# WangFeng18/3d-gaussian-splatting

Measured on NVIDIA H100. Metric: render+backward FPS @1080p (2.4M Gaussians), higher is better.
Workload: dtype f32

## Files before the change

3d-gaussian-splatting_b200/csrc/blend.cu:

```cuda
#include <cstdlib>
#include <type_traits>

#include "internal.h"

namespace {

constexpr int FWD_THREADS = 64;
constexpr int FWD_PX = 4;
constexpr int FWD_STAGES = 2;

template <int FWD_CH>
struct FwdSmem {
  float4 A[FWD_STAGES][FWD_CH];
  float4 C[FWD_STAGES][FWD_CH];
  float2 B[FWD_STAGES][FWD_CH + 2];
  uint64_t full[FWD_STAGES];
};

template <typename SM, int CH>
__device__ __forceinline__ void issue_chunk(SM& sm, int stage, const float4* __restrict__ pA,
                                            const float2* __restrict__ pB, const float4* __restrict__ pC,
                                            int base, int n, int shift) {
  uint32_t bytes_a = (uint32_t)n * 16u;
  uint32_t nb = (uint32_t)(n + shift + 1) & ~1u;
// ... 577 lines not shown
    const float ev = fmaf(-b.x * dy, dy, b.y);                                              \
    _Pragma("unroll") for (int p = 0; p < FWD_PX; ++p) {                                    \
      const float dx = px[p] - a.x;                                                         \
      const float eu = fmaf(a.z, dx, -m1);                                                  \
      const float alpha = gs_ex2(fmaf(-dx, eu, ev));                                        \
      const float w = (T[p] > GS_T_STOP) ? alpha * T[p] : 0.f;                              \
      cr[p] = fmaf(c.x, w, cr[p]);                                                          \
      cg[p] = fmaf(c.y, w, cg[p]);                                                          \
      cb[p] = fmaf(c.z, w, cb[p]);                                                          \
      T[p] -= w;                                                                            \
    }                                                                                       \
  }
    int j = 0;
    bool warp_dead = false;
    for (; j + 4 <= n; j += 4) {
#pragma unroll
      for (int u = 0; u < 4; ++u) GS_FWD_BODY(j + u)
      const bool dead = !(T[0] > GS_T_STOP) && !(T[1] > GS_T_STOP) && !(T[2] > GS_T_STOP) && !(T[3] > GS_T_STOP);
      if (__all_sync(0xffffffffu, dead)) {
        warp_dead = true;
        break;
      }
    }
    if (!warp_dead)
      for (; j < n; ++j) GS_FWD_BODY(j)
#undef GS_FWD_BODY
    const bool dead = !(T[0] > GS_T_STOP) && !(T[1] > GS_T_STOP) && !(T[2] > GS_T_STOP) && !(T[3] > GS_T_STOP);
    const int all_dead = gs_bar_red_and(1, WSF_CONS, dead);
    if (all_dead) {
      consumed = min(cnt, (k + 1) * WS_CH);
      if (tid == 0) {
        sm.consumed_chunks = k + 1;
        sm.stop = 1;
        gs_mbar_arrive(&sm.empty[stage]);
      }
      break;
    }
    if (tid == 0) {
      sm.consumed_chunks = k + 1;
      gs_mbar_arrive(&sm.empty[stage]);
    }
  }
  if (tid == 0 && nchunks > 0) gs_mbar_arrive(&sm.done);
  float4* o = reinterpret_cast<float4*>(image + ((size_t)iy * wp + ix0) * 3);
  o[0] = make_float4(cr[0], cg[0], cb[0], cr[1]);
  o[1] = make_float4(cg[1], cb[1], cr[2], cg[2]);
  o[2] = make_float4(cb[2], cr[3], cg[3], cb[3]);
  if (final_img) {
#pragma unroll
    for (int p = 0; p < FWD_PX; ++p)
      gs_store_final(final_img, ix0 + p, iy, crop.left, crop.top, crop.width, crop.height, cr[p], cg[p], cb[p]);
  }
  if (tile_neff && tid == 0) tile_neff[tile] = consumed;
}

template <int PX, int STAGES_, int RQ_>
struct Bwd2Cfg {
  static constexpr int NT = 256 / PX;
  static constexpr int TPR = GS_TILE / PX;
  static constexpr int RQ = RQ_;
  static constexpr int R = NT / RQ;
  static constexpr int SQ = NT / RQ;
  static constexpr int ROWS = SQ / TPR;
  static constexpr int QS = (SQ * 6 + 31) / 32 * 32 + 32 / RQ;
  static constexpr int IS = RQ * QS + 2 - (RQ * QS) % 32 + ((RQ * QS) % 32 > 2 ? 32 : 0);
  static constexpr int STAGES = STAGES_;
};

template <int PX, int STAGES, int RQ, bool GATHER, int CH>
struct Bwd2Smem : std::conditional<GATHER, GatherRing<CH, STAGES, 4>, WsRing<STAGES>>::type {
  float part[Bwd2Cfg<PX, STAGES, RQ>::R * Bwd2Cfg<PX, STAGES, RQ>::IS];
  float pyt[GS_TILE];
  int valid[2];
};

template <int PX, int STAGES, int RQ, bool GATHER, int CH>
struct Bwd2SmemAux : Bwd2Smem<PX, STAGES, RQ, GATHER, CH> {
  static constexpr int TQS = Bwd2Cfg<PX, STAGES, RQ>::SQ, TIS = Bwd2Cfg<PX, STAGES, RQ>::NT + 1;
  static_assert(Bwd2Cfg<PX, STAGES, RQ>::NT == 32 && TQS * RQ == 32 && TIS % 32 == 1,
                "d_t plane strides are conflict free for one consumer warp only");
  float part_t[Bwd2Cfg<PX, STAGES, RQ>::R * TIS];
};

template <int PX, bool AUX = false>
__device__ __forceinline__ void bwd_row(const float4 a, const float2 b, const float4 c, const float (&px)[PX],
                                        const float py, float (&T)[PX], float (&Rr)[PX], const float (&gr)[PX],
                                        const float (&gg)[PX], const float (&gb)[PX], float2* __restrict__ dst,
                                        const float t = 0.f, const float (*gD)[PX] = nullptr,
                                        const float (*gA)[PX] = nullptr, float* __restrict__ dst_t = nullptr) {
  float s0 = 0.f, sx = 0.f, sxx = 0.f, c0 = 0.f, c1 = 0.f, c2 = 0.f, dt = 0.f;
  const float dy = py - a.y;
  const float m1 = a.w * dy;
  const float ev = fmaf(-b.x * dy, dy, b.y);
#pragma unroll
  for (int p = 0; p < PX; ++p) {
    const float dx = px[p] - a.x;
    const float eu = fmaf(a.z, dx, -m1);
    float alpha = gs_ex2(fmaf(-dx, eu, ev));
    alpha = (T[p] > GS_T_STOP) ? alpha : 0.f;
    const float w = alpha * T[p];
    float gc = fmaf(gr[p], c.x, fmaf(gg[p], c.y, gb[p] * c.z));
    if constexpr (AUX) gc = fmaf((*gD)[p], t, gc + (*gA)[p]);
    Rr[p] = fmaf(-gc, w, Rr[p]);
    const float rc = gs_rcp(1.0000001f - alpha);
    const float dal = fmaf(T[p], gc, -Rr[p] * rc);
    const float e = dal * alpha;
    T[p] -= w;
    const float ex = e * dx;
    s0 += e;
    sx += ex;
    sxx = fmaf(ex, dx, sxx);
    c0 = fmaf(gr[p], w, c0);
    c1 = fmaf(gg[p], w, c1);
    c2 = fmaf(gb[p], w, c2);
    if constexpr (AUX) dt = fmaf((*gD)[p], w, dt);
  }
  dst[0] = make_float2(s0, sx);
  dst[1] = make_float2(sxx, c0);
  dst[2] = make_float2(c1, c2);
  if constexpr (AUX) *dst_t = dt;
}

template <int PX, bool WS, int UNR, int STAGES, int MINB, int RQ, bool GATHER, int CH, bool AUX = false>
__global__ void __launch_bounds__(256 / PX + (WS ? 32 : 0), MINB)
    blend_bwd2_kernel(const float4* __restrict__ pA, const float2* __restrict__ pB, const float4* __restrict__ pC,
                      const GsRec* __restrict__ grec, const uint32_t* __restrict__ ids,
                      const uint32_t* __restrict__ goff, const int* __restrict__ tile_accum, int wp, int hp, int ntx, float fx, float fy,
                      const float* __restrict__ image, const float* __restrict__ grad_image,
                      float* __restrict__ grad_inst, int grad_is_final, GsCrop crop, uint32_t* __restrict__ row_epoch,
                      uint32_t epoch, int* __restrict__ tile_neff_b, const float* __restrict__ aux,
                      const float* __restrict__ grad_aux) {
  using Cfg = Bwd2Cfg<PX, STAGES, RQ>;
  constexpr int NT = Cfg::NT, TPR = Cfg::TPR, R = Cfg::R, SQ = Cfg::SQ, QS = Cfg::QS, IS = Cfg::IS, ROWS = Cfg::ROWS;
  static_assert(IS % 2 == 0 && QS % 2 == 0 && IS % 32 == 2 && QS % 32 == 32 / RQ, "partial buffer strides");
  static_assert(!(WS && GATHER), "the gather path issues its copies from all consumer threads");
  static_assert(GATHER || CH == WS_CH, "the packed ring is sized for CH instances per stage");
  static_assert(!AUX || GATHER, "the aux terms read |p_c| from the gathered records");
  using Smem = typename std::conditional<AUX, Bwd2SmemAux<PX, STAGES, RQ, GATHER, CH>,
                                         Bwd2Smem<PX, STAGES, RQ, GATHER, CH>>::type;
  __shared__ __align__(16) Smem sm;
  const int tile = blockIdx.x;
  const int tid = threadIdx.x, warp = tid >> 5, lane = tid & 31;
  const int start = tile_accum[tile];
  const int cnt = tile_accum[tile + 1] - start;
  if (cnt == 0) return;
  const int nchunks = (cnt + CH - 1) / CH;
  const int tx = tile % ntx, ty = tile / ntx;
  const int shift = start & 1;
  if (tid < GS_TILE) sm.pyt[tid] = gs_pixel_coord(ty * GS_TILE + tid, hp, fy);
  if constexpr (GATHER) {
    if (tid == 0) {
      for (int s = 0; s < STAGES; ++s) gs_mbar_init(&sm.full[s], NT);
      gs_fence_barrier_init();
    }
    __syncthreads();
  } else {
    ws_init<Smem, STAGES>(sm, tid);
    if (WS) {
      if (tid >= NT) {
        if (tid == NT) ws_producer<Smem, STAGES>(sm, pA, pB, pC, start, cnt, nchunks);
        return;
      }
    } else if (tid == 0) {
      for (int k = 0; k < STAGES && k < nchunks; ++k)
        issue_chunk<Smem, CH>(sm, k, pA, pB, pC, start + k * CH, min(CH, cnt - k * CH), shift);
    }
  }
  GatherIds<NT, CH> gid;
  if constexpr (GATHER) {
    for (int k = 0; k < STAGES && k < nchunks; ++k) {
      gid.load(ids, start + k * CH, min(CH, cnt - k * CH), tid);
      gather_issue<Smem, NT, CH, 4>(sm, k, grec, goff, gid, min(CH, cnt - k * CH), tid);
    }
    if (STAGES < nchunks) gid.load(ids, start + STAGES * CH, min(CH, cnt - STAGES * CH), tid);
  }
  const int ix0 = tx * GS_TILE + (tid % TPR) * PX;
  const int iy = ty * GS_TILE + (tid / TPR);
  float px[PX];
#pragma unroll
  for (int p = 0; p < PX; ++p) px[p] = gs_pixel_coord(ix0 + p, wp, fx);
  const float py = sm.pyt[tid / TPR];

  float T[PX], Rr[PX], gr[PX], gg[PX], gb[PX];
  {
    const size_t off = ((size_t)iy * wp + ix0) * 3;
    const float4* im = reinterpret_cast<const float4*>(image + off);
    float gbuf[PX * 3], ibuf[PX * 3];
#pragma unroll
    for (int q = 0; q < PX * 3 / 4; ++q) {
      const float4 i4 = im[q];
      ibuf[4 * q] = i4.x; ibuf[4 * q + 1] = i4.y; ibuf[4 * q + 2] = i4.z; ibuf[4 * q + 3] = i4.w;
    }
    if (!grad_is_final) {
      const float4* gi = reinterpret_cast<const float4*>(grad_image + off);
#pragma unroll
      for (int q = 0; q < PX * 3 / 4; ++q) {
        const float4 g4 = gi[q];
        gbuf[4 * q] = g4.x; gbuf[4 * q + 1] = g4.y; gbuf[4 * q + 2] = g4.z; gbuf[4 * q + 3] = g4.w;
      }
    } else {
#pragma unroll
      for (int p = 0; p < PX; ++p)
        gs_load_final_grad(grad_image, ibuf + 3 * p, ix0 + p, iy, crop.left, crop.top, crop.width, crop.height,
                           gbuf[3 * p], gbuf[3 * p + 1], gbuf[3 * p + 2]);
    }
#pragma unroll
    for (int p = 0; p < PX; ++p) {
      gr[p] = gbuf[3 * p];
      gg[p] = gbuf[3 * p + 1];
      gb[p] = gbuf[3 * p + 2];
      Rr[p] = gr[p] * ibuf[3 * p] + gg[p] * ibuf[3 * p + 1] + gb[p] * ibuf[3 * p + 2];
      T[p] = 1.f;
    }
  }
  float gD[PX], gA[PX];
  if constexpr (AUX) {
    const size_t off = ((size_t)iy * wp + ix0) * 2;
    float abuf[PX * 2], gbuf[PX * 2];
#pragma unroll
    for (int q = 0; q < PX / 2; ++q) {
      const float4 v = reinterpret_cast<const float4*>(aux + off)[q];
      abuf[4 * q] = v.x; abuf[4 * q + 1] = v.y; abuf[4 * q + 2] = v.z; abuf[4 * q + 3] = v.w;
    }
    if (!grad_is_final) {
#pragma unroll
      for (int q = 0; q < PX / 2; ++q) {
        const float4 v = reinterpret_cast<const float4*>(grad_aux + off)[q];
        gbuf[4 * q] = v.x; gbuf[4 * q + 1] = v.y; gbuf[4 * q + 2] = v.z; gbuf[4 * q + 3] = v.w;
      }
    } else {
#pragma unroll
      for (int p = 0; p < PX; ++p) {
        const int x = ix0 + p - crop.left, y = iy - crop.top;
        float2 v = make_float2(0.f, 0.f);
        if (x >= 0 && x < crop.width && y >= 0 && y < crop.height)
          v = *reinterpret_cast<const float2*>(grad_aux + ((size_t)y * crop.width + x) * 2);
        gbuf[2 * p] = v.x;
        gbuf[2 * p + 1] = v.y;
      }
    }
#pragma unroll
    for (int p = 0; p < PX; ++p) {
      gD[p] = gbuf[2 * p];
      gA[p] = gbuf[2 * p + 1];
      Rr[p] = fmaf(gD[p], abuf[2 * p], fmaf(gA[p], abuf[2 * p + 1], Rr[p]));
    }
  }
  float2* const my_part = reinterpret_cast<float2*>(sm.part + (tid / SQ) * QS + (tid % SQ) * 6);
  float* my_part_t = nullptr;
  if constexpr (AUX) my_part_t = sm.part_t + (tid / SQ) * Smem::TQS + (tid % SQ);
  const int ri = tid / RQ, rq = tid % RQ;
  const float2* const red_src = reinterpret_cast<const float2*>(sm.part + ri * IS + rq * QS);

  int consumed = cnt;
  bool finished = false;
  int k = 0;
  for (; k < nchunks && !finished; ++k) {
    const int stage = k % STAGES;
    gs_mbar_wait(&sm.full[stage], (uint32_t)((k / STAGES) & 1));
    const int n = min(CH, cnt - k * CH);
    StageView<GATHER> sv;
    if constexpr (GATHER) {
      sv.R = sm.rec[stage];
      sv.recw = 4;
    } else {
      sv.A = sm.A[stage];
      sv.C = sm.C[stage];
      sv.B = sm.B[stage] + shift;
    }

    for (int sub = 0; sub < n; sub += R) {
      const int nr = min(R, n - sub);
      int j = 0;
      bool wdead = false;
      for (; j + UNR <= nr; j += UNR) {
        if (UNR >= 4 || (j & 3) == 0) {
          bool dead = true;
#pragma unroll
          for (int p = 0; p < PX; ++p) dead = dead && !(T[p] > GS_T_STOP);
          if (__all_sync(0xffffffffu, dead)) {
            wdead = true;
            break;
          }
        }
#pragma unroll
        for (int u = 0; u < UNR; ++u) {
          if constexpr (AUX)
            bwd_row<PX, true>(sv.a(sub + j + u), sv.b(sub + j + u), sv.c(sub + j + u), px, py, T, Rr, gr, gg, gb,
                              my_part + (j + u) * (IS / 2), sv.depth(sub + j + u), &gD, &gA,
                              my_part_t + (j + u) * Smem::TIS);
          else
            bwd_row<PX>(sv.a(sub + j + u), sv.b(sub + j + u), sv.c(sub + j + u), px, py, T, Rr, gr, gg, gb,
                        my_part + (j + u) * (IS / 2));
        }
      }
      if (UNR > 1 && !wdead)
        for (; j < nr; ++j) {
          if constexpr (AUX)
            bwd_row<PX, true>(sv.a(sub + j), sv.b(sub + j), sv.c(sub + j), px, py, T, Rr, gr, gg, gb,
                              my_part + j * (IS / 2), sv.depth(sub + j), &gD, &gA, my_part_t + j * Smem::TIS);
          else
            bwd_row<PX>(sv.a(sub + j), sv.b(sub + j), sv.c(sub + j), px, py, T, Rr, gr, gg, gb, my_part + j * (IS / 2));
        }
      bool dead = true;
#pragma unroll
      for (int p = 0; p < PX; ++p) dead = dead && !(T[p] > GS_T_STOP);
      int all_dead;
      int v0, v1;
      if (NT == 64) {
        if (lane == 0) sm.valid[warp] = j;
        all_dead = gs_bar_red_and(1, NT, dead);
        v0 = sm.valid[0];
        v1 = sm.valid[1];
      } else {
        __syncwarp();
        all_dead = __all_sync(0xffffffffu, dead);
        v0 = v1 = j;
      }
      {
        float S0 = 0.f, Sx = 0.f, Sxx = 0.f, Sy = 0.f, Sxy = 0.f, Syy = 0.f, C0 = 0.f, C1 = 0.f, C2 = 0.f;
        const bool act = ri < nr;
        float4 a = make_float4(0.f, 0.f, 0.f, 0.f);
        float2 b = make_float2(0.f, 0.f);
        if (act) {
          a = sv.a(sub + ri);
          b = sv.b(sub + ri);
        }
        const int vq = (NT == 64 && rq * SQ >= 32) ? v1 : v0;
        if (act && ri < vq) {
#pragma unroll
          for (int r = 0; r < ROWS; ++r) {
            float2 u0 = red_src[(r * TPR) * 3], u1 = red_src[(r * TPR) * 3 + 1], u2 = red_src[(r * TPR) * 3 + 2];
#pragma unroll
            for (int t = 1; t < TPR; ++t) {
              const float2 w0 = red_src[(r * TPR + t) * 3], w1 = red_src[(r * TPR + t) * 3 + 1],
                           w2 = red_src[(r * TPR + t) * 3 + 2];
              u0.x += w0.x; u0.y += w0.y; u1.x += w1.x; u1.y += w1.y; u2.x += w2.x; u2.y += w2.y;
            }
            const float dyr = sm.pyt[ROWS * rq + r] - a.y;
            S0 += u0.x;
            Sx += u0.y;
            Sxx += u1.x;
            C0 += u1.y;
            C1 += u2.x;
            C2 += u2.y;
            Sy = fmaf(dyr, u0.x, Sy);
            Sxy = fmaf(dyr, u0.y, Sxy);
            Syy = fmaf(dyr * dyr, u0.x, Syy);
          }
        }
        float Dt = 0.f;
        if constexpr (AUX) {
          if (act && ri < vq) {
            const float* src = sm.part_t + ri * Smem::TIS + rq * Smem::TQS;
#pragma unroll
            for (int s = 0; s < SQ; ++s) Dt += src[s];
          }
        }
#define GS_RED4(V)                                   \
  V += __shfl_xor_sync(0xffffffffu, V, 1);           \
  V += __shfl_xor_sync(0xffffffffu, V, 2);           \
  if (RQ == 8) V += __shfl_xor_sync(0xffffffffu, V, 4);
        GS_RED4(S0) GS_RED4(Sx) GS_RED4(Sxx) GS_RED4(Sy) GS_RED4(Sxy) GS_RED4(Syy) GS_RED4(C0) GS_RED4(C1) GS_RED4(C2)
        if constexpr (AUX) { GS_RED4(Dt) }
#undef GS_RED4
        if (act) {
          const uint32_t slot = sv.slot(sub + ri, tx, ty);
          float4* out = reinterpret_cast<float4*>(grad_inst + (size_t)slot * GS_GREC);
          if (rq == 0)
            out[0] = make_float4(GS_LN2 * (2.f * a.z * Sx - a.w * Sy), GS_LN2 * (2.f * b.x * Sy - a.w * Sx),
                                 -GS_LN2 * Sxx, GS_LN2 * Sxy);
          else if (rq == 1)
            out[1] = make_float4(-GS_LN2 * Syy, GS_LN2 * S0, C0, C1);
          else if (rq == 2)
            out[2] = make_float4(C2, Dt, 0.f, 0.f);
          else if (rq == 3 && row_epoch)
            row_epoch[slot] = epoch;
        }
      }
      if (NT == 64) gs_bar_sync(1, NT);
      else __syncwarp();
      if (all_dead) {
        consumed = min(cnt, k * CH + sub + nr);
        finished = true;
        break;
      }
    }
    if constexpr (GATHER) {
      if (!finished && k + STAGES < nchunks) {
        const int kn = k + STAGES;
        gather_issue<Smem, NT, CH, 4>(sm, stage, grec, goff, gid, min(CH, cnt - kn * CH), tid);
        if (kn + 1 < nchunks) gid.load(ids, start + (kn + 1) * CH, min(CH, cnt - (kn + 1) * CH), tid);
      }
    } else if (tid == 0) {
      if (WS) {
        sm.consumed_chunks = k + 1;
        if (finished) sm.stop = 1;
        gs_mbar_arrive(&sm.empty[stage]);
      } else if (!finished && k + STAGES < nchunks) {
        const int kn = k + STAGES;
        issue_chunk<Smem, CH>(sm, stage, pA, pB, pC, start + kn * CH, min(CH, cnt - kn * CH), shift);
      }
    }
  }
  if (tid == 0) {
    if constexpr (!GATHER && WS) {
      gs_mbar_arrive(&sm.done);
    } else if (finished) {
      for (int kk = k; kk < nchunks && kk < k + STAGES - 1; ++kk)
        gs_mbar_wait(&sm.full[kk % STAGES], (uint32_t)((kk / STAGES) & 1));
    }
    if (tile_neff_b) tile_neff_b[tile] = consumed;
  }
  if (row_epoch || GATHER) return;
  for (int t = consumed + tid; t < cnt; t += NT) {
    const uint32_t slot = __float_as_uint(pC[start + t].w);
    float4* out = reinterpret_cast<float4*>(grad_inst + (size_t)slot * GS_GREC);
    const float4 z = make_float4(0.f, 0.f, 0.f, 0.f);
    out[0] = z;
    out[1] = z;
    out[2] = z;
  }
}

__global__ void __launch_bounds__(256) legacy_pack_kernel(const float* __restrict__ pos, const float* __restrict__ rgb,
                                                           const float* __restrict__ opa,
                                                           const float* __restrict__ cov, int m,
                                                           float4* __restrict__ pA, float2* __restrict__ pB,
                                                           float4* __restrict__ pC) {
  int i = blockIdx.x * 256 + threadIdx.x;
  if (i >= m) return;
  float4 cv = reinterpret_cast<const float4*>(cov)[i];
  GsConic k = gs_make_conic(cv.x, cv.y, cv.z, cv.w);
  pA[i] = make_float4(pos[3 * i], pos[3 * i + 1], k.ca, k.cb);
  pB[i] = make_float2(k.cc, log2f(opa[i]));
  pC[i] = make_float4(rgb[3 * i], rgb[3 * i + 1], rgb[3 * i + 2], __uint_as_float((uint32_t)i));
}

__global__ void __launch_bounds__(256) legacy_unpack_grads_kernel(const float* __restrict__ grad_inst,
                                                                   const float* __restrict__ opa,
                                                                   const float* __restrict__ cov, int m,
                                                                   float* __restrict__ g_pos,
                                                                   float* __restrict__ g_rgb,
                                                                   float* __restrict__ g_opa,
                                                                   float* __restrict__ g_cov) {
  int i = blockIdx.x * 256 + threadIdx.x;
  if (i >= m) return;
  const float4* row = reinterpret_cast<const float4*>(grad_inst + (size_t)i * GS_GREC);
  float4 v0 = row[0], v1 = row[1], v2 = row[2];
  float4 cv = reinterpret_cast<const float4*>(cov)[i];
  float det = cv.x * cv.w - cv.y * cv.z;
  double pn = 2.0 * (double)det + 1e-14;
  float sc = (float)((double)GS_LOG2E / pn);
  float kk = 2.f * sc * sc / GS_LOG2E;
  float gsc = v0.z * cv.w + v0.w * (cv.y + cv.z) + v1.x * cv.x;
  g_pos[3 * i] = v0.x;
  g_pos[3 * i + 1] = v0.y;
  reinterpret_cast<float4*>(g_cov)[i] = make_float4(v1.x * sc - gsc * kk * cv.w, v0.w * sc + gsc * kk * cv.z,
                                                    v0.w * sc + gsc * kk * cv.y, v0.z * sc - gsc * kk * cv.x);
  g_opa[i] = opa[i] > 0.f ? v1.y / (opa[i] * GS_LN2) : 0.f;
  g_rgb[3 * i] = v1.z;
  g_rgb[3 * i + 1] = v1.w;
  g_rgb[3 * i + 2] = v2.x;
}

__global__ void __launch_bounds__(256) legacy_pack_sh_kernel(const float* __restrict__ pos,
                                                              const float* __restrict__ rgb,
                                                              const float* __restrict__ opa,
                                                              const float* __restrict__ cov, int m, int d, int sw,
// ... 28 lines not shown
  float kk = 2.f * sc * sc / GS_LOG2E;
  float d_ca = row[2], d_cb = row[3], d_cc = row[4];
  float gsc = d_ca * cv.w + d_cb * (cv.y + cv.z) + d_cc * cv.x;
  g_pos[3 * i] = row[0];
  g_pos[3 * i + 1] = row[1];
  reinterpret_cast<float4*>(g_cov)[i] = make_float4(d_cc * sc - gsc * kk * cv.w, d_cb * sc + gsc * kk * cv.z,
                                                    d_cb * sc + gsc * kk * cv.y, d_ca * sc - gsc * kk * cv.x);
  g_opa[i] = opa[i] > 0.f ? row[5] / (opa[i] * GS_LN2) : 0.f;
  for (int q = 0; q < d; ++q) g_rgb[(size_t)i * d + q] = row[6 + q];
}

struct LegacyWs {
  float4* pA;
  float2* pB;
  float4* pC;
  float* grad_inst;
};

inline size_t align_up(size_t x, size_t a) { return (x + a - 1) / a * a; }

inline size_t legacy_ws_layout(int m, int d, LegacyWs* ws, char* base) {
  size_t off = 0;
  size_t mm = (size_t)(m > 0 ? m : 0);
  size_t crow = d == 3 ? 16 : (size_t)gs_sh_stream_width(d) * 4;
  size_t grow = d == 3 ? (size_t)GS_GREC * 4 : (size_t)gs_sh_grad_width(d) * 4;
  if (ws) ws->pA = reinterpret_cast<float4*>(base + off);
  off += align_up(mm * 16, 256);
  if (ws) ws->pC = reinterpret_cast<float4*>(base + off);
  off += align_up(mm * crow + 16, 256);
  if (ws) ws->pB = reinterpret_cast<float2*>(base + off);
  off += align_up((mm + 2) * 8, 256);
  if (ws) ws->grad_inst = reinterpret_cast<float*>(base + off);
  off += align_up(mm * grow, 256);
  return off;
}

}

cudaError_t gs_launch_blend_fwd(const float4* pA, const float2* pB, const float4* pC, const GsRec* grec,
                                const uint32_t* ids, const int* tile_accum, const GsFrameGeom& g, float* image,
                                int* tile_neff, float* final_img, const GsCrop& crop, cudaStream_t st,
                                const GsAuxOut* aux) {
  const GsTuning& tn = gs_tuning();
  const bool gather = grec != nullptr;
  if (aux) {
    blend_fwd_kernel<128, 4, true, true><<<g.n_tiles, 64, 0, st>>>(pA, pB, pC, grec, ids, tile_accum, g.wp, g.hp, g.ntx,
                                                                  g.fx, g.fy, image, tile_neff, final_img, crop, *aux);
    return cudaGetLastError();
  }
  if (!gather && tn.fwd_kernel != 0) {
    blend_fwd_ws_kernel<<<g.n_tiles, WSF_CONS + 32, 0, st>>>(pA, pB, pC, tile_accum, g.wp, g.hp, g.ntx, g.fx, g.fy, image,
                                                             tile_neff, final_img, crop);
    return cudaGetLastError();
  }
  const int ch = tn.fwd_ch;
#define GS_FWD_LAUNCH(CH, PX, GA)                                                                                   \
  blend_fwd_kernel<CH, PX, GA><<<g.n_tiles, 256 / PX, 0, st>>>(pA, pB, pC, grec, ids, tile_accum, g.wp, g.hp, g.ntx, \
                                                               g.fx, g.fy, image, tile_neff, final_img, crop, GsAuxOut{})
#define GS_FWD_CH(PX, GA)                     \
  if (ch == 64) GS_FWD_LAUNCH(64, PX, GA);    \
  else if (ch == 256) GS_FWD_LAUNCH(256, PX, GA); \
  else GS_FWD_LAUNCH(128, PX, GA)
  if (gather) {
    if (tn.fwd_px == 8) { GS_FWD_CH(8, true); } else { GS_FWD_CH(4, true); }
  } else {
    if (tn.fwd_px == 8) { GS_FWD_CH(8, false); } else { GS_FWD_CH(4, false); }
  }
#undef GS_FWD_CH
#undef GS_FWD_LAUNCH
  return cudaGetLastError();
}

cudaError_t gs_launch_blend_bwd(const float4* pA, const float2* pB, const float4* pC, const GsRec* grec,
                                const uint32_t* ids, const uint32_t* goff, const int* tile_accum, const GsFrameGeom& g,
                                const float* image,
                                const float* grad_image, float* grad_inst, int grad_is_final, const GsCrop& crop,
                                uint32_t* row_epoch, uint32_t epoch, int* tile_neff_b, cudaStream_t st,
                                const float* aux, const float* grad_aux) {
  const GsTuning& tn = gs_tuning();
  const bool gather = grec != nullptr;
  if (gather && !row_epoch) return cudaErrorInvalidValue;
  if (grad_aux) {
    if (!gather || !aux) return cudaErrorInvalidValue;
    blend_bwd2_kernel<8, false, 4, 3, 10, 4, true, 32, true><<<g.n_tiles, 32, 0, st>>>(
        pA, pB, pC, grec, ids, goff, tile_accum, g.wp, g.hp, g.ntx, g.fx, g.fy, image, grad_image, grad_inst,
        grad_is_final, crop, row_epoch, epoch, tile_neff_b, aux, grad_aux);
    return cudaGetLastError();
  }
  if (tn.bwd_kernel != 0 || gather) {
#define GS_BWD2C(PX, WS, UNR, ST, MINB, RQ, GA, CH)                                                                 \
  blend_bwd2_kernel<PX, WS, UNR, ST, MINB, RQ, GA, CH><<<g.n_tiles, 256 / PX + (WS ? 32 : 0), 0, st>>>(              \
      pA, pB, pC, grec, ids, goff, tile_accum, g.wp, g.hp, g.ntx, g.fx, g.fy, image, grad_image, grad_inst,          \
      grad_is_final,                                                                                                 \
      crop, row_epoch, epoch, tile_neff_b, nullptr, nullptr)
#define GS_BWD2(PX, WS, UNR, ST, MINB, RQ, GA) GS_BWD2C(PX, WS, UNR, ST, MINB, RQ, GA, 64)
    const int key = ((((tn.bwd_px * 10 + tn.bwd_ws) * 10 + tn.bwd_unroll) * 10 + tn.bwd_stages) * 10 + tn.bwd_rq) * 100 +
                    tn.bwd_minb;
    if (gather && tn.bwd_ch == 32) {
      switch (key) {
        case 8022416: GS_BWD2C(8, false, 2, 2, 16, 4, true, 32); break;
        case 8023416: GS_BWD2C(8, false, 2, 3, 16, 4, true, 32); break;
        case 8042410: GS_BWD2C(8, false, 4, 2, 10, 4, true, 32); break;
        case 8043410: GS_BWD2C(8, false, 4, 3, 10, 4, true, 32); break;
        default: return gs_tuning().strict ? cudaErrorInvalidValue : (GS_BWD2C(8, false, 4, 3, 10, 4, true, 32), cudaGetLastError());
      }
      return cudaGetLastError();
    }
    if (gather) {
      switch (key) {
        case 8012410: GS_BWD2(8, false, 1, 2, 10, 4, true); break;
        case 8022416: GS_BWD2(8, false, 2, 2, 16, 4, true); break;
        case 8022410: GS_BWD2(8, false, 2, 2, 10, 4, true); break;
        case 8042410: GS_BWD2(8, false, 4, 2, 10, 4, true); break;
        case 8023416: GS_BWD2(8, false, 2, 3, 16, 4, true); break;
        case 8012416: GS_BWD2(8, false, 1, 2, 16, 4, true); break;
        case 8012420: GS_BWD2(8, false, 1, 2, 20, 4, true); break;
        case 8012820: GS_BWD2(8, false, 1, 2, 20, 8, true); break;
        case 8013416: GS_BWD2(8, false, 1, 3, 16, 4, true); break;
        case 4012401: GS_BWD2(4, false, 1, 2, 1, 4, true); break;
        case 4042401: GS_BWD2(4, false, 4, 2, 1, 4, true); break;
        default: return gs_tuning().strict ? cudaErrorInvalidValue : (GS_BWD2(8, false, 2, 2, 16, 4, true), cudaGetLastError());
      }
      return cudaGetLastError();
    }
    switch (key) {
      case 4113401: GS_BWD2(4, true, 1, 3, 1, 4, false); break;
      case 4143408: GS_BWD2(4, true, 4, 3, 8, 4, false); break;
      case 4012401: GS_BWD2(4, false, 1, 2, 1, 4, false); break;
      case 4042401: GS_BWD2(4, false, 4, 2, 1, 4, false); break;
      case 4042810: GS_BWD2(4, false, 4, 2, 10, 8, false); break;
      case 8012410: GS_BWD2(8, false, 1, 2, 10, 4, false); break;
      case 8012416: GS_BWD2(8, false, 1, 2, 16, 4, false); break;
      case 8012420: GS_BWD2(8, false, 1, 2, 20, 4, false); break;
      case 8013416: GS_BWD2(8, false, 1, 3, 16, 4, false); break;
      case 8022416: GS_BWD2(8, false, 2, 2, 16, 4, false); break;
      case 8022410: GS_BWD2(8, false, 2, 2, 10, 4, false); break;
      case 8042410: GS_BWD2(8, false, 4, 2, 10, 4, false); break;
      case 8012816: GS_BWD2(8, false, 1, 2, 16, 8, false); break;
      case 8012820: GS_BWD2(8, false, 1, 2, 20, 8, false); break;
      case 8112410: GS_BWD2(8, true, 1, 2, 10, 4, false); break;
      case 8012424: GS_BWD2(8, false, 1, 2, 24, 4, false); break;
      case 8012824: GS_BWD2(8, false, 1, 2, 24, 8, false); break;
      default: return gs_tuning().strict ? cudaErrorInvalidValue : (GS_BWD2(8, false, 2, 2, 16, 4, false), cudaGetLastError());
    }
#undef GS_BWD2
#undef GS_BWD2C
    return cudaGetLastError();
  }
  const int warps = tn.bwd_px == 8 ? 1 : 2;
  const int ch = 64;
#define GS_BWD_LAUNCH(W, CH)                                                                                         \
  blend_bwd_kernel<W, CH><<<g.n_tiles, 32 * W, 0, st>>>(pA, pB, pC, tile_accum, g.wp, g.hp, g.ntx, g.fx, g.fy, image, \
                                                        grad_image, grad_inst, grad_is_final, crop, row_epoch, epoch, \
                                                        tile_neff_b)
  if (warps == 1) GS_BWD_LAUNCH(1, 64);
  else if (ch == 32) GS_BWD_LAUNCH(2, 32);
  else if (ch == 128) GS_BWD_LAUNCH(2, 128);
  else GS_BWD_LAUNCH(2, 64);
#undef GS_BWD_LAUNCH
  return cudaGetLastError();
}

int gs_blend_aux_supported(int d, bool forward, bool backward) {
  const GsTuning& tn = gs_tuning();
  if (!tn.gather)
    return gs_set_error_msg(GS_ERR_UNSUPPORTED, "depth / alpha / background: the packed path (gs_tune(\"gather\", 0)) has no aux kernel");
  if (d != 3) {
    if (backward && (gs_sh_tc_mode(d) & 6) == 6)
      return gs_set_error_msg(GS_ERR_UNSUPPORTED,
                              "depth / alpha gradients: the two-pixel tensor-core SH backward (sh_tc bit 2) has no aux kernel");
    return 0;
  }
  if (forward && (tn.fwd_kernel != 0 || tn.fwd_ch != 128 || tn.fwd_px != 4))
    return gs_set_error_msg(GS_ERR_UNSUPPORTED,
                            "depth / alpha / background: only the shipped forward blend knobs (fwd_kernel 0, fwd_ch 128, fwd_px 4) have an aux kernel");
  if (backward && (tn.bwd_kernel == 0 || tn.bwd_px != 8 || tn.bwd_ws != 0 || tn.bwd_unroll != 4 || tn.bwd_stages != 3 ||
                   tn.bwd_rq != 4 || tn.bwd_minb != 10 || tn.bwd_ch != 32))
    return gs_set_error_msg(GS_ERR_UNSUPPORTED,
                            "depth / alpha gradients: only the shipped backward blend knobs have an aux kernel");
  return 0;
}

extern "C" size_t gs_draw_workspace_bytes(int m, int d) {
  if (d != 3 && gs_sh_basis_count(d) == 0) return 0;
  return legacy_ws_layout(m, d, nullptr, nullptr);
}

static int check_draw_args(const char* fn, int m, int d, int wp, int hp, int weight_normalize, int sigmoid,
// ... 102 lines not shown
```

3d-gaussian-splatting_b200/csrc/internal.h:

```cpp
#pragma once
#include <cuda_runtime.h>
#include <stdint.h>

#include "../../include/gs_b200.h"
#include "project.cuh"

#define GS_GREC 12

struct GsFrameGeom {
  int width, height, wp, hp, ntx, nty, n_tiles;
  float fx, fy;
};

struct GsCrop {
  int left, top, width, height;
};

struct GsAuxOut {
  float bg[3];
  float* aux;
  float* aux_final;
};

#ifdef __CUDACC__
__device__ __forceinline__ void gs_store_aux(const GsAuxOut& ax, int ix, int iy, int wp, const GsCrop& crop,
                                             float depth, float alpha) {
  if (ax.aux) *reinterpret_cast<float2*>(ax.aux + ((size_t)iy * wp + ix) * 2) = make_float2(depth, alpha);
  const int x = ix - crop.left, y = iy - crop.top;
  if (ax.aux_final && x >= 0 && x < crop.width && y >= 0 && y < crop.height)
    *reinterpret_cast<float2*>(ax.aux_final + ((size_t)y * crop.width + x) * 2) = make_float2(depth, alpha);
}
template <int PX>
__device__ __forceinline__ void gs_load_aux_grad(const float* __restrict__ aux, const float* __restrict__ grad_aux,
                                                 int grad_is_final, int ix0, int iy, int wp, const GsCrop& crop,
                                                 float (&gD)[PX], float (&gA)[PX], float (&R)[PX]) {
#pragma unroll
  for (int p = 0; p < PX; ++p) {
    const size_t off = ((size_t)iy * wp + ix0 + p) * 2;
    const float2 da = *reinterpret_cast<const float2*>(aux + off);
    float2 g = make_float2(0.f, 0.f);
    if (!grad_is_final) {
      g = *reinterpret_cast<const float2*>(grad_aux + off);
    } else {
      const int x = ix0 + p - crop.left, y = iy - crop.top;
      if (x >= 0 && x < crop.width && y >= 0 && y < crop.height)
        g = *reinterpret_cast<const float2*>(grad_aux + ((size_t)y * crop.width + x) * 2);
    }
    gD[p] = g.x;
    gA[p] = g.y;
    R[p] = fmaf(g.x, da.x, fmaf(g.y, da.y, R[p]));
  }
}
#endif

struct GsRayPtrs {
  const float *rays_o, *lefttop, *dx, *dy;
};

struct GsTuning {
  int fwd_kernel;
  int fwd_ch;
  int bwd_kernel;
  int bwd_px;
  int bwd_ws;
  int bwd_unroll;
  int bwd_stages;
  int bwd_minb;
  int bwd_rq;
  int fwd_px;
  int bwd_ch;
  int strict;
  int gather;
  int sh_tc;
};
GsTuning& gs_tuning();

void gs_count_launch(int n = 1);

int gs_sh_basis_count(int d);
int gs_sh_stream_width(int d);
int gs_sh_grad_width(int d);
int gs_sh_tc_mode(int d);
cudaError_t gs_launch_blend_sh_fwd(const float4* pA, const float2* pB, const float* pS, const GsRec* grec,
                                   const float* rgb, const uint32_t* ids, const uint32_t* goff , int d,
                                   const int* tile_accum,
                                   const GsFrameGeom& g, const GsRayPtrs& r, float* image, int* tile_neff,
                                   float* final_img, const GsCrop& crop, cudaStream_t st,
                                   const GsAuxOut* aux = nullptr );
cudaError_t gs_launch_blend_sh_bwd(const float4* pA, const float2* pB, const float* pS, const GsRec* grec,
                                   const float* rgb, const uint32_t* ids, const uint32_t* goff , int d,
                                   const int* tile_accum,
                                   const GsFrameGeom& g, const GsRayPtrs& r, const float* image,
                                   const float* grad_image, float* grad_inst, int grad_is_final, const GsCrop& crop,
                                   uint32_t* row_epoch, uint32_t epoch, int* tile_neff_b, cudaStream_t st,
                                   const float* aux = nullptr, const float* grad_aux = nullptr );

cudaError_t gs_launch_blend_sh_fwd_tc(const GsRec* grec, const float* rgb, const uint32_t* ids, int d,
                                      const int* tile_accum, const GsFrameGeom& g, const GsRayPtrs& r, float* image,
                                      int* tile_neff, float* final_img, const GsCrop& crop, cudaStream_t st,
                                      const GsAuxOut* aux = nullptr);
cudaError_t gs_launch_blend_sh_bwd_tc(const GsRec* grec, const float* rgb, const uint32_t* ids, const uint32_t* goff, int d,
                                      const int* tile_accum, const GsFrameGeom& g, const GsRayPtrs& r, const float* image,
                                      const float* grad_image, float* grad_inst, int grad_is_final, const GsCrop& crop,
                                      uint32_t* row_epoch, uint32_t epoch, int* tile_neff_b, cudaStream_t st,
                                      const float* aux = nullptr, const float* grad_aux = nullptr);

cudaError_t gs_launch_fused_project(const float* pos, const float* rgb, const float* opa, const float* quat,
                                    const float* scale, int n, int d, int scale_act, const GsCam& cam,
                                    const GsTileGrid& grid, float near_plane, float half_w, float half_h,
                                    GsRec* rec, uint32_t* count, uint32_t* dkey, int64_t* mask,
                                    unsigned int* n_visible, cudaStream_t st,
                                    bool sh_gaussian = false );

struct GsGradPush {
  float* bucket;
  float* staging[GS_MAX_PEERS];
  uint32_t per;
  int rank, world;
};

cudaError_t gs_launch_fused_project_bwd(const float* pos, const float* rgb, const float* opa, const float* quat,
                                        const float* scale, int n, int d, int scale_act, const GsCam& cam,
                                        float near_plane, float half_w, float half_h, const uint32_t* offsets_g,
                                        const uint32_t* count, const float* grad_inst, const uint32_t* row_epoch, uint32_t epoch,
                                        float* g_pos, float* g_rgb, float* g_opa,
                                        float* g_quat, float* g_scale, const GsGradPush& push, cudaStream_t st,
                                        bool depth_grad = false ,
                                        bool sh_gaussian = false );
size_t gs_cam_grad_workspace_bytes(int n);
cudaError_t gs_launch_fused_project_bwd_cam(const float* pos, const float* rgb, const float* opa, const float* quat,
                                            const float* scale, int n, int d, int scale_act, const GsCam& cam,
                                            float near_plane, float half_w, float half_h, const uint32_t* offsets_g,
                                            const uint32_t* count, const float* grad_inst, const uint32_t* row_epoch,
                                            uint32_t epoch, float* g_pos, float* g_rgb, float* g_opa, float* g_quat,
                                            float* g_scale, float* cam_part, float* grad_cam, cudaStream_t st,
                                            bool depth_grad, bool sh_gaussian);

cudaError_t gs_launch_emit_keys(const GsRec* rec, const uint32_t* perm, const uint32_t* offsets_sorted, int n, int ntx,
                                void* keys, int key_bytes, uint32_t* vals, cudaStream_t st);
cudaError_t gs_launch_tile_ranges(const void* keys, int key_bytes, long long m, int n_tiles, int* tile_accum,
                                  cudaStream_t st);

cudaError_t gs_launch_pack_sorted(const void* keys, int key_bytes, const uint32_t* vals, long long m, int n_tiles,
                                  int ntx, const GsRec* rec, const uint32_t* offsets_g, float4* pA, float2* pB, float4* pC,
                                  int* tile_accum, cudaStream_t st);

cudaError_t gs_launch_pack_sorted_sh(const void* keys, int key_bytes, const uint32_t* vals, long long m, int n_tiles,
                                     int ntx, const GsRec* rec, const uint32_t* offsets_g, const float* rgb, int d, int sw,
                                     float4* pA, float2* pB, float* pS, int* tile_accum, cudaStream_t st);
cudaError_t gs_launch_iota(uint32_t* out, int n, cudaStream_t st);

cudaError_t gs_launch_blend_fwd(const float4* pA, const float2* pB, const float4* pC, const GsRec* grec,
                                const uint32_t* ids, const int* tile_accum, const GsFrameGeom& g, float* image,
                                int* tile_neff, float* final_img, const GsCrop& crop, cudaStream_t st,
                                const GsAuxOut* aux = nullptr );

// ... 10 lines not shown
```

3d-gaussian-splatting_b200/csrc/render.cu:

```cuda
#include <cub/device/device_radix_sort.cuh>
#include <cub/device/device_scan.cuh>
#include <cub/iterator/counting_input_iterator.cuh>
#include <cub/iterator/transform_input_iterator.cuh>

#include <cmath>
#include <cstdio>
#include <cstdlib>
#include <cstring>
#include <new>

#include "internal.h"

struct GsCountInSortedOrder {
  const uint32_t* count;
  const uint32_t* perm;
  uint32_t n;
  __host__ __device__ __forceinline__ uint32_t operator()(uint32_t i) const { return i < n ? count[perm[i]] : 0u; }
};

static thread_local char g_err[512] = {0};

int gs_set_error(cudaError_t e, const char* what) {
  snprintf(g_err, sizeof(g_err), "CUDA error %d (%s) at %s", (int)e, cudaGetErrorString(e), what);
  return (int)e;
}
int gs_set_error_msg(int code, const char* what) {
  snprintf(g_err, sizeof(g_err), "%s", what);
  return code;
}
extern "C" const char* gs_last_error(void) { return g_err; }
extern "C" int gs_abi_version(void) { return 2; }

static int tune_env(const char* name, int dflt) {
  const char* e = getenv(name);
  return e ? atoi(e) : dflt;
}
GsTuning& gs_tuning() {
  static GsTuning t = {tune_env("GS_TUNE_FWD_KERNEL", 0),  tune_env("GS_TUNE_FWD_CH", 128),   tune_env("GS_TUNE_BWD_KERNEL", 1),
                       tune_env("GS_TUNE_BWD_PX", 8),      tune_env("GS_TUNE_BWD_WS", 0),     tune_env("GS_TUNE_BWD_UNROLL", 4),
                       tune_env("GS_TUNE_BWD_STAGES", 3),  tune_env("GS_TUNE_BWD_MINB", 10),  tune_env("GS_TUNE_BWD_RQ", 4),
                       tune_env("GS_TUNE_FWD_PX", 4),      tune_env("GS_TUNE_BWD_CH", 32),    tune_env("GS_TUNE_STRICT", 0),
                       tune_env("GS_TUNE_GATHER", 1),      tune_env("GS_TUNE_SH_TC", -1)};
  return t;
}
extern "C" int gs_tune(const char* name, int value) {
  if (!name) return gs_set_error_msg(GS_ERR_INVALID_ARG, "gs_tune: null name");
  GsTuning& t = gs_tuning();
  struct { const char* k; int* v; } tab[] = {{"fwd_kernel", &t.fwd_kernel}, {"fwd_ch", &t.fwd_ch},
                                             {"bwd_kernel", &t.bwd_kernel}, {"bwd_px", &t.bwd_px},
                                             {"bwd_ws", &t.bwd_ws},         {"bwd_unroll", &t.bwd_unroll},
                                             {"bwd_stages", &t.bwd_stages}, {"bwd_minb", &t.bwd_minb},
                                             {"bwd_rq", &t.bwd_rq},         {"fwd_px", &t.fwd_px},
                                             {"gather", &t.gather},         {"bwd_ch", &t.bwd_ch},
                                             {"strict", &t.strict},         {"sh_tc", &t.sh_tc}};
  for (auto& e : tab)
    if (!strcmp(e.k, name)) {
      *e.v = value;
      return 0;
    }
  return gs_set_error_msg(GS_ERR_INVALID_ARG, "gs_tune: unknown knob");
}

#include <atomic>
static std::atomic<unsigned long long> g_launches{0};
void gs_count_launch(int n) { g_launches.fetch_add((unsigned long long)n, std::memory_order_relaxed); }
extern "C" unsigned long long gs_kernel_launches(void) { return g_launches.load(std::memory_order_relaxed); }

struct GsAllocator {
  gs_alloc_fn alloc = nullptr;
  gs_free_fn free = nullptr;
  void* user = nullptr;
};
static thread_local const GsAllocator* g_cur_alloc = nullptr;

struct DevBuf {
  void* p = nullptr;
  size_t cap = 0;
  const GsAllocator* owner = nullptr;
  void drop(cudaStream_t st, bool sync) {
    if (!p) return;
    if (owner && owner->free) {
      owner->free(p, owner->user);
    } else {
      if (sync) cudaStreamSynchronize(st);
      cudaFree(p);
    }
    p = nullptr;
    cap = 0;
  }
  cudaError_t reserve(size_t bytes, cudaStream_t st) {
    if (bytes <= cap) return cudaSuccess;
    drop(st, true);
    size_t want = bytes + bytes / 8 + 256;
    const GsAllocator* a = g_cur_alloc;
    if (a && a->alloc) {
      p = a->alloc(want, a->user, (gs_stream_t)st);
      if (!p) return cudaErrorMemoryAllocation;
      owner = a;
    } else {
      cudaError_t e = cudaMalloc(&p, want);
      if (e != cudaSuccess) return e;
      owner = nullptr;
    }
    cap = want;
    return cudaSuccess;
  }
  void release() { drop(nullptr, false); }
  template <typename T>
  T* as() const { return static_cast<T*>(p); }
};

struct gs_ctx {
  int device = 0;
  GsAllocator allocator{};
  DevBuf rec, count, offsets, dkey_in, dkey_out, perm, iota, offsets_g;
  size_t iota_n = 0;
  DevBuf keys_in, keys_out, vals_in, vals_out, pA, pB, pC, grad_inst, row_epoch;
  uint32_t epoch = 0;
  DevBuf tile_accum, tile_neff, tile_neff_b, cub_tmp, counters, img_dev, gimg_dev, rays;
  DevBuf cam_part;
  float* host_rays = nullptr;
  unsigned long long* host_m = nullptr;
  cudaEvent_t ev_m = nullptr;
  bool have_forward = false, have_backward = false, gather = false;
  bool have_aux = false;
  bool sh_gaussian = false;
  int n = 0, d = 3, scale_act = 0;
  long long m = 0;
  GsCam cam{};
  GsTileGrid grid{};
  GsFrameGeom geom{};
  float near_plane = 0.f, half_w = 0.f, half_h = 0.f;
  int64_t* mask_ptr = nullptr;
  bool timing = false;
  cudaEvent_t ev[GS_N_STAGES + 2] = {};
  bool ev_ok = false;
  bool ev_fwd_valid = false, ev_bwd_valid = false;
// ... 624 lines not shown
```

Before: 438.2.

## Repack live pixels across lanes in backward blend to shrink per-lane work

Adds a warp-level compaction step to the backward blend kernel. Once enough pixels have saturated transmittance, the still-live pixel states are redistributed across lanes so each lane holds 4, 2 or 1 of them, and the inner loop runs with a smaller compile-time pixel count. Each lane's row y is stored so the reduction can still form the y moments. This targets wasted work on dead pixels late in long tiles, at the cost of shuffles, shared-memory traffic, four template instantiations (more code and possible register pressure) and a non-unrolled loop for the reduced widths. It is enabled by default through a new tuning knob.

```diff
diff --git a/3d-gaussian-splatting_b200/csrc/blend.cu b/3d-gaussian-splatting_b200/csrc/blend.cu
--- a/3d-gaussian-splatting_b200/csrc/blend.cu
+++ b/3d-gaussian-splatting_b200/csrc/blend.cu
@@ -683,7 +683,7 @@
   float part_t[Bwd2Cfg<PX, STAGES, RQ>::R * TIS];
 };
 
-template <int PX, bool AUX = false>
+template <int PX, bool AUX = false, int NP = PX>
 __device__ __forceinline__ void bwd_row(const float4 a, const float2 b, const float4 c, const float (&px)[PX],
                                         const float py, float (&T)[PX], float (&Rr)[PX], const float (&gr)[PX],
                                         const float (&gg)[PX], const float (&gb)[PX], float2* __restrict__ dst,
@@ -694,7 +694,7 @@
   const float m1 = a.w * dy;
   const float ev = fmaf(-b.x * dy, dy, b.y);
 #pragma unroll
-  for (int p = 0; p < PX; ++p) {
+  for (int p = 0; p < NP; ++p) {
     const float dx = px[p] - a.x;
     const float eu = fmaf(a.z, dx, -m1);
     float alpha = gs_ex2(fmaf(-dx, eu, ev));
@@ -722,7 +722,104 @@
   if constexpr (AUX) *dst_t = dt;
 }
 
-template <int PX, bool WS, int UNR, int STAGES, int MINB, int RQ, bool GATHER, int CH, bool AUX = false>
+template <int SQ, int QS>
+__device__ __forceinline__ int bwd_lane_y(int l) {
+  static_assert(QS - SQ * 6 >= SQ, "a part has room for its source lanes' row y");
+  return (l / SQ) * QS + SQ * 6 + l % SQ;
+}
+
+constexpr int RP_ROWLIVE = 2048, RP_SRC = RP_ROWLIVE + GS_TILE, RP_CNT = RP_SRC + 32, RP_ROW = RP_CNT + 32,
+              RP_PY = RP_ROW + 32, RP_END = RP_PY + 32;
+template <int PX, bool AUX, int SQ, int QS>
+__device__ __forceinline__ void bwd_repack(float* __restrict__ st, const float* __restrict__ pyt, int lane, int& S,
+                                           int& prow, float& py, float (&px)[PX], float (&T)[PX], float (&Rr)[PX],
+                                           float (&gr)[PX], float (&gg)[PX], float (&gb)[PX], float (&gD)[PX],
+                                           float (&gA)[PX]) {
+  int* const rowlive = reinterpret_cast<int*>(st + RP_ROWLIVE);
+  int* const lsrc = reinterpret_cast<int*>(st + RP_SRC);
+  int* const lcnt = reinterpret_cast<int*>(st + RP_CNT);
+  int* const lrow = reinterpret_cast<int*>(st + RP_ROW);
+  float* const lpy = st + RP_PY;
+  int c = 0;
+#pragma unroll
+  for (int p = 0; p < PX; ++p) c += T[p] > GS_T_STOP ? 1 : 0;
+  if (__reduce_add_sync(0xffffffffu, c) > 16 * S) return;
+  if (lane < GS_TILE) rowlive[lane] = 0;
+  __syncwarp();
+  if (c) atomicAdd(&rowlive[prow], c);
+  __syncwarp();
+  const int live = lane < GS_TILE ? rowlive[lane] : 0;
+  int ns = S;
+  while (ns > 1 && __reduce_add_sync(0xffffffffu, (live + ns / 2 - 1) / (ns / 2)) <= 32) ns /= 2;
+  if (ns == S) return;
+
+  int incl = c;
+#pragma unroll
+  for (int o = 1; o < 32; o <<= 1) {
+    const int t = __shfl_up_sync(0xffffffffu, incl, o);
+    if (lane >= o) incl += t;
+  }
+  int pos = incl - c;
+#pragma unroll
+  for (int p = 0; p < PX; ++p)
+    if (T[p] > GS_T_STOP) {
+      st[pos] = px[p];
+      st[256 + pos] = T[p];
+      st[512 + pos] = Rr[p];
+      st[768 + pos] = gr[p];
+      st[1024 + pos] = gg[p];
+      st[1280 + pos] = gb[p];
+      if constexpr (AUX) {
+        st[1536 + pos] = gD[p];
+        st[1792 + pos] = gA[p];
+      }
+      ++pos;
+    }
+  lsrc[lane] = 0;
+  lcnt[lane] = 0;
+  lrow[lane] = GS_TILE;
+  lpy[lane] = 0.f;
+  const int nl = (live + ns - 1) / ns;
+  int sc = (nl << 16) | live;
+#pragma unroll
+  for (int o = 1; o < 32; o <<= 1) {
+    const int t = __shfl_up_sync(0xffffffffu, sc, o);
+    if (lane >= o) sc += t;
+  }
+  sc -= (nl << 16) | live;
+  __syncwarp();
+  for (int q = 0; q < nl; ++q) {
+    const int l = (sc >> 16) + q;
+    lsrc[l] = (sc & 0xffff) + q * ns;
+    lcnt[l] = min(ns, live - q * ns);
+    lrow[l] = lane;
+    lpy[l] = pyt[lane];
+  }
+  __syncwarp();
+  const int src = lsrc[lane], n = lcnt[lane];
+  prow = lrow[lane];
+  py = lpy[lane];
+#pragma unroll
+  for (int p = 0; p < PX; ++p) {
+    const bool v = p < n;
+    px[p] = v ? st[src + p] : 0.f;
+    T[p] = v ? st[256 + src + p] : 0.f;
+    Rr[p] = v ? st[512 + src + p] : 0.f;
+    gr[p] = v ? st[768 + src + p] : 0.f;
+    gg[p] = v ? st[1024 + src + p] : 0.f;
+    gb[p] = v ? st[1280 + src + p] : 0.f;
+    if constexpr (AUX) {
+      gD[p] = v ? st[1536 + src + p] : 0.f;
+      gA[p] = v ? st[1792 + src + p] : 0.f;
+    }
+  }
+  __syncwarp();
+  st[bwd_lane_y<SQ, QS>(lane)] = py;
+  S = ns;
+}
+
+template <int PX, bool WS, int UNR, int STAGES, int MINB, int RQ, bool GATHER, int CH, bool AUX = false,
+          bool REPACK = false>
 __global__ void __launch_bounds__(256 / PX + (WS ? 32 : 0), MINB)
     blend_bwd2_kernel(const float4* __restrict__ pA, const float2* __restrict__ pB, const float4* __restrict__ pC,
                       const GsRec* __restrict__ grec, const uint32_t* __restrict__ ids,
@@ -737,6 +834,8 @@
   static_assert(!(WS && GATHER), "the gather path issues its copies from all consumer threads");
   static_assert(GATHER || CH == WS_CH, "the packed ring is sized for CH instances per stage");
   static_assert(!AUX || GATHER, "the aux terms read |p_c| from the gathered records");
+  static_assert(!REPACK || (NT == 32 && PX == 8), "the repack deals one warp's 256 pixels into slots of at most 8");
+  static_assert(!REPACK || R * IS >= RP_END, "the partial buffer holds the repack's planes and tables");
   using Smem = typename std::conditional<AUX, Bwd2SmemAux<PX, STAGES, RQ, GATHER, CH>,
                                          Bwd2Smem<PX, STAGES, RQ, GATHER, CH>>::type;
   __shared__ __align__(16) Smem sm;
@@ -780,7 +879,8 @@
   float px[PX];
 #pragma unroll
   for (int p = 0; p < PX; ++p) px[p] = gs_pixel_coord(ix0 + p, wp, fx);
-  const float py = sm.pyt[tid / TPR];
+  float py = sm.pyt[tid / TPR];
+  int S = PX, prow = tid / TPR;
 
   float T[PX], Rr[PX], gr[PX], gg[PX], gb[PX];
   {
@@ -872,37 +972,54 @@
 
     for (int sub = 0; sub < n; sub += R) {
       const int nr = min(R, n - sub);
-      int j = 0;
-      bool wdead = false;
-      for (; j + UNR <= nr; j += UNR) {
-        if (UNR >= 4 || (j & 3) == 0) {
-          bool dead = true;
-#pragma unroll
-          for (int p = 0; p < PX; ++p) dead = dead && !(T[p] > GS_T_STOP);
-          if (__all_sync(0xffffffffu, dead)) {
-            wdead = true;
-            break;
+      auto phase1 = [&](auto np) -> int {
+        constexpr int NP = decltype(np)::value, U = NP == PX ? UNR : 1;
+        int j = 0;
+        bool wdead = false;
+#pragma unroll 1
+        for (; j + U <= nr; j += U) {
+          if (U >= 4 || (j & 3) == 0) {
+            bool dead = true;
+#pragma unroll
+            for (int p = 0; p < PX; ++p) dead = dead && !(T[p] > GS_T_STOP);
+            if (__all_sync(0xffffffffu, dead)) {
+              wdead = true;
+              break;
+            }
+          }
+#pragma unroll
+          for (int u = 0; u < U; ++u) {
+            if constexpr (AUX)
+              bwd_row<PX, true, NP>(sv.a(sub + j + u), sv.b(sub + j + u), sv.c(sub + j + u), px, py, T, Rr, gr, gg,
+                                    gb, my_part + (j + u) * (IS / 2), sv.depth(sub + j + u), &gD, &gA,
+                                    my_part_t + (j + u) * Smem::TIS);
+            else
+              bwd_row<PX, false, NP>(sv.a(sub + j + u), sv.b(sub + j + u), sv.c(sub + j + u), px, py, T, Rr, gr, gg,
+                                     gb, my_part + (j + u) * (IS / 2));
           }
         }
-#pragma unroll
-        for (int u = 0; u < UNR; ++u) {
-          if constexpr (AUX)
-            bwd_row<PX, true>(sv.a(sub + j + u), sv.b(sub + j + u), sv.c(sub + j + u), px, py, T, Rr, gr, gg, gb,
-                              my_part + (j + u) * (IS / 2), sv.depth(sub + j + u), &gD, &gA,
-                              my_part_t + (j + u) * Smem::TIS);
-          else
-            bwd_row<PX>(sv.a(sub + j + u), sv.b(sub + j + u), sv.c(sub + j + u), px, py, T, Rr, gr, gg, gb,
-                        my_part + (j + u) * (IS / 2));
+        if (U > 1 && !wdead)
+          for (; j < nr; ++j) {
+            if constexpr (AUX)
+              bwd_row<PX, true, NP>(sv.a(sub + j), sv.b(sub + j), sv.c(sub + j), px, py, T, Rr, gr, gg, gb,
+                                    my_part + j * (IS / 2), sv.depth(sub + j), &gD, &gA, my_part_t + j * Smem::TIS);
+            else
+              bwd_row<PX, false, NP>(sv.a(sub + j), sv.b(sub + j), sv.c(sub + j), px, py, T, Rr, gr, gg, gb,
+                                     my_part + j * (IS / 2));
+          }
+        return j;
+      };
+      int j;
+      if constexpr (REPACK) {
+        switch (S) {
+          case 8: j = phase1(std::integral_constant<int, 8>{}); break;
+          case 4: j = phase1(std::integral_constant<int, 4>{}); break;
+          case 2: j = phase1(std::integral_constant<int, 2>{}); break;
+          default: j = phase1(std::integral_constant<int, 1>{}); break;
         }
-      }
-      if (UNR > 1 && !wdead)
-        for (; j < nr; ++j) {
-          if constexpr (AUX)
-            bwd_row<PX, true>(sv.a(sub + j), sv.b(sub + j), sv.c(sub + j), px, py, T, Rr, gr, gg, gb,
-                              my_part + j * (IS / 2), sv.depth(sub + j), &gD, &gA, my_part_t + j * Smem::TIS);
-          else
-            bwd_row<PX>(sv.a(sub + j), sv.b(sub + j), sv.c(sub + j), px, py, T, Rr, gr, gg, gb, my_part + j * (IS / 2));
-        }
+      } else {
+        j = phase1(std::integral_constant<int, PX>{});
+      }
       bool dead = true;
 #pragma unroll
       for (int p = 0; p < PX; ++p) dead = dead && !(T[p] > GS_T_STOP);
@@ -928,7 +1045,23 @@
           b = sv.b(sub + ri);
         }
         const int vq = (NT == 64 && rq * SQ >= 32) ? v1 : v0;
-        if (act && ri < vq) {
+        if (REPACK && act && ri < vq && S < PX) {
+#pragma unroll
+          for (int s = 0; s < SQ; ++s) {
+            const float2 w0 = red_src[s * 3], w1 = red_src[s * 3 + 1], w2 = red_src[s * 3 + 2];
+            float dyl = 0.f;
+            if constexpr (REPACK) dyl = sm.part[bwd_lane_y<SQ, QS>(rq * SQ + s)] - a.y;
+            S0 += w0.x;
+            Sx += w0.y;
+            Sxx += w1.x;
+            C0 += w1.y;
+            C1 += w2.x;
+            C2 += w2.y;
+            Sy = fmaf(dyl, w0.x, Sy);
+            Sxy = fmaf(dyl, w0.y, Sxy);
+            Syy = fmaf(dyl * dyl, w0.x, Syy);
+          }
+        } else if (act && ri < vq) {
 #pragma unroll
           for (int r = 0; r < ROWS; ++r) {
             float2 u0 = red_src[(r * TPR) * 3], u1 = red_src[(r * TPR) * 3 + 1], u2 = red_src[(r * TPR) * 3 + 2];
@@ -986,6 +1119,8 @@
         finished = true;
         break;
       }
+      if constexpr (REPACK)
+        if (S > 1) bwd_repack<PX, AUX, SQ, QS>(sm.part, sm.pyt, lane, S, prow, py, px, T, Rr, gr, gg, gb, gD, gA);
     }
     if constexpr (GATHER) {
       if (!finished && k + STAGES < nchunks) {
@@ -1180,9 +1315,13 @@
   if (gather && !row_epoch) return cudaErrorInvalidValue;
   if (grad_aux) {
     if (!gather || !aux) return cudaErrorInvalidValue;
-    blend_bwd2_kernel<8, false, 4, 3, 10, 4, true, 32, true><<<g.n_tiles, 32, 0, st>>>(
-        pA, pB, pC, grec, ids, goff, tile_accum, g.wp, g.hp, g.ntx, g.fx, g.fy, image, grad_image, grad_inst,
-        grad_is_final, crop, row_epoch, epoch, tile_neff_b, aux, grad_aux);
+#define GS_BWD2_AUX(RP)                                                                                            \
+  blend_bwd2_kernel<8, false, 4, 3, 10, 4, true, 32, true, RP><<<g.n_tiles, 32, 0, st>>>(                           \
+      pA, pB, pC, grec, ids, goff, tile_accum, g.wp, g.hp, g.ntx, g.fx, g.fy, image, grad_image, grad_inst,         \
+      grad_is_final, crop, row_epoch, epoch, tile_neff_b, aux, grad_aux)
+    if (tn.blend_repack) GS_BWD2_AUX(true);
+    else GS_BWD2_AUX(false);
+#undef GS_BWD2_AUX
     return cudaGetLastError();
   }
   if (tn.bwd_kernel != 0 || gather) {
@@ -1195,13 +1334,24 @@
     const int key = ((((tn.bwd_px * 10 + tn.bwd_ws) * 10 + tn.bwd_unroll) * 10 + tn.bwd_stages) * 10 + tn.bwd_rq) * 100 +
                     tn.bwd_minb;
     if (gather && tn.bwd_ch == 32) {
+#define GS_BWD2_SHIPPED()                                                                                          \
+  if (tn.blend_repack)                                                                                             \
+    blend_bwd2_kernel<8, false, 4, 3, 10, 4, true, 32, false, true><<<g.n_tiles, 32, 0, st>>>(                      \
+        pA, pB, pC, grec, ids, goff, tile_accum, g.wp, g.hp, g.ntx, g.fx, g.fy, image, grad_image, grad_inst,       \
+        grad_is_final, crop, row_epoch, epoch, tile_neff_b, nullptr, nullptr);                                     \
+  else                                                                                                             \
+    GS_BWD2C(8, false, 4, 3, 10, 4, true, 32)
       switch (key) {
         case 8022416: GS_BWD2C(8, false, 2, 2, 16, 4, true, 32); break;
         case 8023416: GS_BWD2C(8, false, 2, 3, 16, 4, true, 32); break;
         case 8042410: GS_BWD2C(8, false, 4, 2, 10, 4, true, 32); break;
-        case 8043410: GS_BWD2C(8, false, 4, 3, 10, 4, true, 32); break;
-        default: return gs_tuning().strict ? cudaErrorInvalidValue : (GS_BWD2C(8, false, 4, 3, 10, 4, true, 32), cudaGetLastError());
-      }
+        case 8043410: GS_BWD2_SHIPPED(); break;
+        default:
+          if (gs_tuning().strict) return cudaErrorInvalidValue;
+          GS_BWD2_SHIPPED();
+          break;
+      }
+#undef GS_BWD2_SHIPPED
       return cudaGetLastError();
     }
     if (gather) {
diff --git a/3d-gaussian-splatting_b200/csrc/internal.h b/3d-gaussian-splatting_b200/csrc/internal.h
--- a/3d-gaussian-splatting_b200/csrc/internal.h
+++ b/3d-gaussian-splatting_b200/csrc/internal.h
@@ -72,6 +72,7 @@
   int strict;
   int gather;
   int sh_tc;
+  int blend_repack;
 };
 GsTuning& gs_tuning();
 
diff --git a/3d-gaussian-splatting_b200/csrc/render.cu b/3d-gaussian-splatting_b200/csrc/render.cu
--- a/3d-gaussian-splatting_b200/csrc/render.cu
+++ b/3d-gaussian-splatting_b200/csrc/render.cu
@@ -40,7 +40,7 @@
                        tune_env("GS_TUNE_BWD_PX", 8),      tune_env("GS_TUNE_BWD_WS", 0),     tune_env("GS_TUNE_BWD_UNROLL", 4),
                        tune_env("GS_TUNE_BWD_STAGES", 3),  tune_env("GS_TUNE_BWD_MINB", 10),  tune_env("GS_TUNE_BWD_RQ", 4),
                        tune_env("GS_TUNE_FWD_PX", 4),      tune_env("GS_TUNE_BWD_CH", 32),    tune_env("GS_TUNE_STRICT", 0),
-                       tune_env("GS_TUNE_GATHER", 1),      tune_env("GS_TUNE_SH_TC", -1)};
+                       tune_env("GS_TUNE_GATHER", 1),      tune_env("GS_TUNE_SH_TC", -1),     tune_env("GS_TUNE_BLEND_REPACK", 1)};
   return t;
 }
 extern "C" int gs_tune(const char* name, int value) {
@@ -52,7 +52,8 @@
                                              {"bwd_stages", &t.bwd_stages}, {"bwd_minb", &t.bwd_minb},
                                              {"bwd_rq", &t.bwd_rq},         {"fwd_px", &t.fwd_px},
                                              {"gather", &t.gather},         {"bwd_ch", &t.bwd_ch},
-                                             {"strict", &t.strict},         {"sh_tc", &t.sh_tc}};
+                                             {"strict", &t.strict},         {"sh_tc", &t.sh_tc},
+                                             {"blend_repack", &t.blend_repack}};
   for (auto& e : tab)
     if (!strcmp(e.k, name)) {
       *e.v = value;
```

Measured after the change: 455.4, median of 6. 3.9% higher.
